# VatsalPandey0202/PointCloudRegistration

Hardware: AMD Instinct MI355X
Metric: TOF/PC pairs/sec (8192 pts) (higher is better)
Workload: dtype f32 xyz/features; f64 RANSAC/ICP; 1-term f16 MFMA screen (certified bound), f16x3-split MFMA screen for the rows it leaves, f64 exact re-rank; 1 GPU; C4: batch of augmented TOF/PC pairs (featNN+RANSAC+ICP+Chamfer); pairs_total=256, pairs_per_gpu=256, points=8192, feature_dim=32, streams_per_gpu=1, ransac=d=0.04 mutual n=3 edge0.9 dist0.04 (100000,0.999), icp=d=0.02 (1e-6,1e-6,30), parallelism=pair-sharded x1, inputs=resident in HBM (--full: host_resident is the PCIe-inclusive rate)

## Files before the change

### pointcloudregistration_amd/csrc/featnn_thresh.h

```cpp
#pragma once
#include <stdint.h>
#include <string.h>

#if defined(__HIPCC__)
#define PCR_THRESH_HD __host__ __device__
#else
#define PCR_THRESH_HD
#endif

namespace pcr {

PCR_THRESH_HD inline uint32_t thresh_bits_up(double t) {
    if (!(t == t)) return 0x7f800000u;
    if (!(t > 0.0)) return 0u;
    const float f = (float)t;
    uint32_t b;
    memcpy(&b, &f, sizeof(b));
    return (double)f < t ? b + 1u : b;
}

}
```

### pointcloudregistration_amd/csrc/featnn_thresh.hip

```cpp
#include "featnn_v5.h"
#include "featnn_thresh.h"
#include <stdlib.h>
#include <algorithm>
#include <cstdio>

namespace pcr {
namespace {

__device__ unsigned g_thresh_stat[2][3];

template <int S, bool kIdx>
__global__ __launch_bounds__(512) void featnn_thresh9(RowArgs5 a) {
    constexpr int NM = 2 * S + 1, NB = S, W = 8, RT = 2;
    const int nbp = gridDim.x / (8 * ((a.P + 7) >> 3));
    const int bid = blockIdx.x, xcd = bid & 7, slot = bid >> 3;
    const int p = (slot / nbp) * 8 + xcd, sl = slot % nbp;
    if (p >= a.P) return;
    const int nr = min(a.rcount[p], a.Rmax);
    const int m = count_of(a.n_cols, p, a.Cmax);
    const int nst = (((m + 31) >> 5) + 1) >> 1;
    const int nsl = min(nbp, nst);
    if (nr <= 0 || sl >= nsl) return;
    const int s0 = (int)((long long)nst * sl / nsl), s1 = (int)((long long)nst * (sl + 1) / nsl);
    const int wid = threadIdx.x >> 6, l = threadIdx.x & 63, h = l >> 5;
    const int ntl = (nr + 31) >> 5;
    const int *rl = a.rlist + (size_t)p * a.Rmax;
    const f16x8 *bimg = a.Bp + (size_t)p * a.ntc * NM * 64 + l;
    const float *ctp = a.cct + (size_t)p * a.ntc * 32;
    auto load = [&](int st, f16x8 (&Bf)[2][NB], f32x16 (&Cf)[2]) {
#pragma unroll
        for (int u = 0; u < 2; ++u) {
#pragma unroll
            for (int c = 0; c < NB; ++c) Bf[u][c] = bimg[((size_t)(2 * st + u) * NM + c) * 64];
            Cf[u] = colterms(ctp + (size_t)(2 * st + u) * 32, h);
        }
    };
    for (int t0 = wid * RT; t0 < ntl; t0 += W * RT) {
        size_t o[RT];
        unsigned B1[RT], thr[RT], am[RT];
        bool live[RT];
        int nh[RT];
        f16x8 A[RT][NB];
#pragma unroll
        for (int t = 0; t < RT; ++t) {
            const int k = (t0 + t) * 32 + (l & 31);
            const bool valid = k < nr;
            const int row = valid ? rl[k] : 0;
            o[t] = (size_t)p * a.Rmax + row;
            B1[t] = valid ? a.rec[o[t]].y : 0x7f800000u;
            thr[t] = 0u;
            live[t] = false;
            if (valid && B1[t] < 0x7f800000u) {
                const double bnd = row_bound_ct(a, p, row, a.rre[(size_t)p * a.ntr * 32 + row], 16 * S);
                thr[t] = thresh_bits_up((double)__uint_as_float(B1[t]) + bnd * (1.0 + 0x1p-20));
                live[t] = thr[t] < 0x7f800000u;
            }
            row_operand1<S>(a, p, row, valid, h, A[t]);
            am[t] = 0xffffffffu;
            nh[t] = 0;
        }
        f16x8 Bf[2][NB];
        f32x16 Cf[2];
        load(s0, Bf, Cf);
        for (int st = s0; st < s1; ++st) {
            f16x8 Bn[2][NB];
            f32x16 Cn[2];
            load(st + 1 < s1 ? st + 1 : st, Bn, Cn);
            f32x16 acc[RT][2];
#pragma unroll
            for (int c = 0; c < NB; ++c)
#pragma unroll
                for (int u = 0; u < 2; ++u)
#pragma unroll
                    for (int t = 0; t < RT; ++t)
                        acc[t][u] = __builtin_amdgcn_mfma_f32_32x32x16_f16(Bf[u][c], A[t][c],
                                                                           c == 0 ? Cf[u] : acc[t][u], 0, 0, 0);
#pragma unroll
            for (int t = 0; t < RT; ++t)
#pragma unroll
                for (int u = 0; u < 2; ++u) {
                    unsigned long long any = 0ull;
#pragma unroll
                    for (int r = 0; r < 16; ++r) any |= __ballot(fbits(acc[t][u][r]) <= thr[t]);
                    if (any == 0ull) continue;
#pragma unroll
                    for (int r = 0; r < 16; ++r) {
                        const unsigned v = fbits(acc[t][u][r]);
                        const int col = 32 * (2 * st + u) + 8 * (r >> 2) + 4 * h + (r & 3);
                        if (v <= thr[t] && live[t] && col < m) {
                            if (kIdx && v == B1[t]) am[t] = umin2(am[t], (unsigned)col);
                            if (nh[t] <= kThreshK) {
                                const unsigned pos = atomicAdd(reinterpret_cast<unsigned *>(a.rec + o[t]), 1u);
                                if (pos < (unsigned)kThreshK) a.cand[o[t] * kThreshK + pos] = col;
                            }
                            ++nh[t];
                        }
                    }
                }
#pragma unroll
            for (int u = 0; u < 2; ++u) {
#pragma unroll
                for (int c = 0; c < NB; ++c) Bf[u][c] = Bn[u][c];
                Cf[u] = Cn[u];
            }
        }
#pragma unroll
        for (int t = 0; t < RT; ++t)
            if (kIdx && am[t] != 0xffffffffu) atomicMin(reinterpret_cast<unsigned *>(a.rec + o[t]) + 2, am[t]);
    }
}

template <int DV, bool kIdx>
__global__ __launch_bounds__(256) void featnn_exact_cand(RowArgs5 a) {
    const int p = blockIdx.y;
    const int nr = min(a.rcount[p], a.Rmax);
    if (nr <= 0) return;
    if (blockIdx.x == 0 && threadIdx.x == 0) atomicAdd(a.fbctr + (kIdx ? 0 : 1), (unsigned long long)nr);
    const int m = count_of(a.n_cols, p, a.Cmax);
    const int *rl = a.rlist + (size_t)p * a.Rmax;
    const int c = threadIdx.x & 7, rr = threadIdx.x >> 3, D = a.D;
    const float4 open = make_float4(__builtin_inff(), __builtin_inff(), __builtin_inff(), 0.0f);
    for (int k0 = blockIdx.x * 32; k0 < nr; k0 += gridDim.x * 32) {
        const bool act = k0 + rr < nr;
        const int row = act ? rl[k0 + rr] : 0;
        const size_t o = (size_t)p * a.Rmax + row;
        const uint4 rc = act ? a.rec[o] : make_uint4(0u, 0x7f800000u, 0u, 1u);
        const int cnt = (int)min(rc.x, (unsigned)kThreshK + 1u);
        double best = __builtin_inf();
        int bj = 0x7fffffff;
        if (act && m > 0 && c < cnt && cnt <= kThreshK && rc.y < 0x7f800000u) {
            const int j = a.cand[o * kThreshK + c];
            const float *q = a.Xr + o * D, *y = a.Xc + ((size_t)p * a.Cmax + j) * D;
            float qf[DV], yf[DV];
            if (D == DV && (((uintptr_t)q | (uintptr_t)y) & 15) == 0) {
#pragma unroll
                for (int k = 0; k < DV; k += 4) {
                    const float4 u = *reinterpret_cast<const float4 *>(q + k), w = *reinterpret_cast<const float4 *>(y + k);
                    qf[k] = u.x; qf[k + 1] = u.y; qf[k + 2] = u.z; qf[k + 3] = u.w;
                    yf[k] = w.x; yf[k + 1] = w.y; yf[k + 2] = w.z; yf[k + 3] = w.w;
                }
            } else {
#pragma unroll
                for (int k = 0; k < DV; ++k) {
                    qf[k] = k < D ? q[k] : 0.0f;
                    yf[k] = k < D ? y[k] : 0.0f;
                }
            }
            double acc = 0.0;
#pragma unroll
            for (int k = 0; k < DV; ++k) {
                const double df = (double)qf[k] - (double)yf[k];
                acc = acc + df * df;
            }
            if (acc < best) { best = acc; bj = j; }
        }
#pragma unroll
        for (int x = 1; x < 8; x <<= 1) {
            const double ob = __shfl_xor(best, x, 64);
            const int oj = __shfl_xor(bj, x, 64);
            if (ob < best || (ob == best && oj < bj)) { best = ob; bj = oj; }
        }
        if (c != 0 || !act) continue;
        if (m == 0) {
            if constexpr (kIdx) {
                a.nn[o] = 0;
                a.nns[o] = 0;
                a.v[o] = __builtin_inf();
                a.e[o] = 0.0f;
            } else {
                a.wq[o] = open;
            }
            continue;
        }
        if constexpr (kIdx) a.nns[o] = rc.z < (unsigned)m ? (int)rc.z : 0;
        const bool over = bj == 0x7fffffff;
        if (a.dbg) {
            atomicAdd(&g_thresh_stat[kIdx ? 0 : 1][0], 1u);
            atomicMax(&g_thresh_stat[kIdx ? 0 : 1][1], rc.x);
            if (over) atomicAdd(&g_thresh_stat[kIdx ? 0 : 1][2], 1u);
        }
        if constexpr (kIdx) {
            if (over) {
                a.llist[(size_t)p * a.Rmax + atomicAdd(a.lcount + p, 1)] = row;
            } else {
                const double sc = (double)__uint_as_float(a.sc[p]);
                a.nn[o] = bj;
                a.v[o] = best * sc * sc;
                a.e[o] = 0.0f;
            }
        } else {
            a.wq[o] = open;
            if (!over) {
                a.nn[o] = bj;
                a.used[(size_t)p * (a.Rmax + 1) + row] = 2;
            }
        }
    }
}

}

static int thresh_blocks_per_pair(int P) {
    static const int forced = [] {
        const char *e = getenv("PCR_THRESH_SLICES");
        return e ? atoi(e) : 0;
    }();
    if (forced >= 1 && forced <= 128) return forced;
    return std::max(4, std::min(32, 1024 / std::max(P, 1)));
}

template <bool kIdx>
int launch_thresh9(const RowArgs5 &r0, int S, hipStream_t s) {
    RowArgs5 r = r0;
    static const bool dbg = getenv("PCR_THRESH_DEBUG") != nullptr;
    r.dbg = dbg ? 1 : 0;
    int rc = fallback_counter(&r.fbctr);
    if (rc != PCR_OK) return rc;
    const int nbp = thresh_blocks_per_pair(r.P);
    const dim3 grid((unsigned)(8LL * nbp * cdiv(r.P, 8)));
    if (S == 1) hipLaunchKernelGGL((featnn_thresh9<1, kIdx>), grid, dim3(512), 0, s, r);
    else hipLaunchKernelGGL((featnn_thresh9<2, kIdx>), grid, dim3(512), 0, s, r);
    PCR_LAUNCH_CHECK();
    const dim3 eg(std::min(8, cdiv(r.Rmax, 32)), r.P);
    if (S == 1) hipLaunchKernelGGL((featnn_exact_cand<16, kIdx>), eg, dim3(256), 0, s, r);
    else hipLaunchKernelGGL((featnn_exact_cand<32, kIdx>), eg, dim3(256), 0, s, r);
    PCR_LAUNCH_CHECK();
    if (dbg) {
        unsigned st[2][3];
        PCR_HIP_CHECK(hipStreamSynchronize(s));
        PCR_HIP_CHECK(hipMemcpyFromSymbol(st, HIP_SYMBOL(g_thresh_stat), sizeof(st)));
        const int d = kIdx ? 0 : 1;
        fprintf(stderr, "thresh pass %d: listed %u, max candidates %u, to the exact rescan %u\n", d + 1, st[d][0],
                st[d][1], st[d][2]);
        const unsigned z[3] = {0, 0, 0};
        PCR_HIP_CHECK(hipMemcpyToSymbol(HIP_SYMBOL(g_thresh_stat), z, sizeof(z), sizeof(z) * d));
    }
    return PCR_OK;
}

template int launch_thresh9<true>(const RowArgs5 &, int, hipStream_t);
template int launch_thresh9<false>(const RowArgs5 &, int, hipStream_t);

}
```

Measured before the change: 48730 pairs/s.

## Stage column tiles in LDS via async global_load_lds and batch candidate hits locally

The threshold-screen kernel now stages groups of column B-fragments and column terms into double-buffered shared memory with async global-to-LDS loads, so the eight waves of a block share one copy instead of each loading from global memory. Candidate hits are counted and stored in per-row LDS slots and flushed to global memory with one atomic per row per row-block, replacing a global atomic per hit. The hit scan first reduces each half of the accumulator to a minimum before balloting. The default number of blocks per pair also drops (256/P instead of 1024/P, minimum 1). This adds large LDS use and block-wide barriers, which may reduce occupancy.

```diff
diff --git a/pointcloudregistration_amd/csrc/featnn_thresh.h b/pointcloudregistration_amd/csrc/featnn_thresh.h
--- a/pointcloudregistration_amd/csrc/featnn_thresh.h
+++ b/pointcloudregistration_amd/csrc/featnn_thresh.h
@@ -19,4 +19,10 @@
     return (double)f < t ? b + 1u : b;
 }
 
+PCR_THRESH_HD inline int thresh_flush_count(uint32_t base, uint32_t local, int K) {
+    if (base >= (uint32_t)K) return 0;
+    const uint32_t room = (uint32_t)K - base;
+    return (int)(local < room ? local : room);
 }
+
+}
diff --git a/pointcloudregistration_amd/csrc/featnn_thresh.hip b/pointcloudregistration_amd/csrc/featnn_thresh.hip
--- a/pointcloudregistration_amd/csrc/featnn_thresh.hip
+++ b/pointcloudregistration_amd/csrc/featnn_thresh.hip
@@ -3,15 +3,42 @@
 #include <stdlib.h>
 #include <algorithm>
 #include <cstdio>
+#include <type_traits>
 
 namespace pcr {
 namespace {
 
 __device__ unsigned g_thresh_stat[2][3];
 
+#ifndef PCR_THRESH_G
+#define PCR_THRESH_G 16
+#endif
+#ifndef PCR_THRESH_PF
+#define PCR_THRESH_PF 1
+#endif
+constexpr int kThreshG = PCR_THRESH_G;
+
+__device__ __forceinline__ unsigned lds_add_rtn(unsigned addr, unsigned v) {
+    unsigned r;
+    asm volatile("ds_add_rtn_u32 %0, %1, %2\n\ts_waitcnt lgkmcnt(0)" : "=v"(r) : "v"(addr), "v"(v) : "memory");
+    return r;
+}
+__device__ __forceinline__ void lds_store(unsigned addr, int v) {
+    asm volatile("ds_write_b32 %0, %1\n\ts_waitcnt lgkmcnt(0)" : : "v"(addr), "v"(v) : "memory");
+}
+
 template <int S, bool kIdx>
 __global__ __launch_bounds__(512) void featnn_thresh9(RowArgs5 a) {
-    constexpr int NM = 2 * S + 1, NB = S, W = 8, RT = 2;
+    constexpr int NM = 2 * S + 1, NB = S, W = 8, RT = 2, G = kThreshG, GS = G / 2;
+    constexpr int kT = G * NB * 64;
+    constexpr int kRows = W * RT * 32;
+    static_assert(G % 2 == 0 && kRows == 512, "whole steps; the flush is one row per thread");
+    __shared__ __attribute__((aligned(16))) f16x8 Bs0[kT];
+    __shared__ __attribute__((aligned(16))) f16x8 Bs1[kT];
+    __shared__ __attribute__((aligned(16))) float Cs0[G * 32];
+    __shared__ __attribute__((aligned(16))) float Cs1[G * 32];
+    __shared__ unsigned hcnt[kRows];
+    __shared__ int hslot[kRows * kThreshK];
     const int nbp = gridDim.x / (8 * ((a.P + 7) >> 3));
     const int bid = blockIdx.x, xcd = bid & 7, slot = bid >> 3;
     const int p = (slot / nbp) * 8 + xcd, sl = slot % nbp;
@@ -22,28 +49,55 @@
     const int nsl = min(nbp, nst);
     if (nr <= 0 || sl >= nsl) return;
     const int s0 = (int)((long long)nst * sl / nsl), s1 = (int)((long long)nst * (sl + 1) / nsl);
+    const int ngr = (s1 - s0 + GS - 1) / GS;
     const int wid = threadIdx.x >> 6, l = threadIdx.x & 63, h = l >> 5;
     const int ntl = (nr + 31) >> 5;
     const int *rl = a.rlist + (size_t)p * a.Rmax;
     const f16x8 *bimg = a.Bp + (size_t)p * a.ntc * NM * 64 + l;
-    const float *ctp = a.cct + (size_t)p * a.ntc * 32;
-    auto load = [&](int st, f16x8 (&Bf)[2][NB], f32x16 (&Cf)[2]) {
-#pragma unroll
-        for (int u = 0; u < 2; ++u) {
-#pragma unroll
-            for (int c = 0; c < NB; ++c) Bf[u][c] = bimg[((size_t)(2 * st + u) * NM + c) * 64];
-            Cf[u] = colterms(ctp + (size_t)(2 * st + u) * 32, h);
+    const float *ctp = a.cct + (size_t)p * a.ntc * 32 + l;
+    auto issue = [&](auto bufc_, int grp) {
+        f16x8 *Bs = decltype(bufc_)::value ? Bs1 : Bs0;
+        float *Cs = decltype(bufc_)::value ? Cs1 : Cs0;
+        const int sg = s0 + grp * GS;
+        for (int c = wid; c < G * NB + GS; c += W) {
+            if (c >= G * NB) {
+                const int j = c - G * NB;
+                if (sg + j < s1)
+                    __builtin_amdgcn_global_load_lds(
+                        (const __attribute__((address_space(1))) void *)(ctp + (size_t)(sg + j) * 64),
+                        (__attribute__((address_space(3))) void *)(Cs + j * 64),
+                        4, 0, 0);
+                continue;
+            }
+            const int g = c / NB, cc = c - g * NB;
+            if (sg + (g >> 1) < s1)
+                __builtin_amdgcn_global_load_lds(
+                    (const __attribute__((address_space(1))) void *)(bimg + ((size_t)(2 * sg + g) * NM + cc) * 64),
+                    (__attribute__((address_space(3))) void *)(Bs + c * 64), 16, 0, 0);
         }
     };
-    for (int t0 = wid * RT; t0 < ntl; t0 += W * RT) {
+    auto min8 = [](const f32x16 &x, int q) {
+        unsigned c = umin2(umin2(fbits(x[8 * q]), fbits(x[8 * q + 1])), fbits(x[8 * q + 2]));
+        c = umin2(umin2(c, fbits(x[8 * q + 3])), fbits(x[8 * q + 4]));
+        c = umin2(umin2(c, fbits(x[8 * q + 5])), fbits(x[8 * q + 6]));
+        return umin2(c, fbits(x[8 * q + 7]));
+    };
+    for (int tb = 0; tb < ntl; tb += W * RT) {
+        hcnt[threadIdx.x] = 0u;
+        issue(std::integral_constant<int, 0>{}, 0);
+        const int nt = tb + wid + W < ntl ? 2 : (tb + wid < ntl ? 1 : 0);
         size_t o[RT];
         unsigned B1[RT], thr[RT], am[RT];
         bool live[RT];
-        int nh[RT];
+        int nh[RT], lr[RT];
+        unsigned ca[RT], sa[RT];
         f16x8 A[RT][NB];
 #pragma unroll
         for (int t = 0; t < RT; ++t) {
-            const int k = (t0 + t) * 32 + (l & 31);
+            lr[t] = (t * W + wid) * 32 + (l & 31);
+            ca[t] = (unsigned)(uintptr_t)(hcnt + lr[t]);
+            sa[t] = (unsigned)(uintptr_t)(hslot + lr[t] * kThreshK);
+            const int k = tb * 32 + lr[t];
             const bool valid = k < nr;
             const int row = valid ? rl[k] : 0;
             o[t] = (size_t)p * a.Rmax + row;
@@ -59,54 +113,98 @@
             am[t] = 0xffffffffu;
             nh[t] = 0;
         }
-        f16x8 Bf[2][NB];
-        f32x16 Cf[2];
-        load(s0, Bf, Cf);
-        for (int st = s0; st < s1; ++st) {
-            f16x8 Bn[2][NB];
-            f32x16 Cn[2];
-            load(st + 1 < s1 ? st + 1 : st, Bn, Cn);
-            f32x16 acc[RT][2];
-#pragma unroll
-            for (int c = 0; c < NB; ++c)
-#pragma unroll
-                for (int u = 0; u < 2; ++u)
-#pragma unroll
-                    for (int t = 0; t < RT; ++t)
-                        acc[t][u] = __builtin_amdgcn_mfma_f32_32x32x16_f16(Bf[u][c], A[t][c],
-                                                                           c == 0 ? Cf[u] : acc[t][u], 0, 0, 0);
-#pragma unroll
-            for (int t = 0; t < RT; ++t)
+        auto sweep = [&](auto ntc_, auto bufc_, int grp) {
+            constexpr int NT = decltype(ntc_)::value;
+            const f16x8 *Bs = decltype(bufc_)::value ? Bs1 : Bs0;
+            const float *Cb = decltype(bufc_)::value ? Cs1 : Cs0;
+            const int sg = s0 + grp * GS, ns = min(GS, s1 - sg);
+            const f16x8 *Bb = Bs + l;
+            auto load = [&](int j, f16x8 (&Bf)[2][NB], f32x16 (&Cf)[2]) {
 #pragma unroll
                 for (int u = 0; u < 2; ++u) {
-                    unsigned long long any = 0ull;
-#pragma unroll
-                    for (int r = 0; r < 16; ++r) any |= __ballot(fbits(acc[t][u][r]) <= thr[t]);
-                    if (any == 0ull) continue;
-#pragma unroll
-                    for (int r = 0; r < 16; ++r) {
-                        const unsigned v = fbits(acc[t][u][r]);
-                        const int col = 32 * (2 * st + u) + 8 * (r >> 2) + 4 * h + (r & 3);
-                        if (v <= thr[t] && live[t] && col < m) {
-                            if (kIdx && v == B1[t]) am[t] = umin2(am[t], (unsigned)col);
-                            if (nh[t] <= kThreshK) {
-                                const unsigned pos = atomicAdd(reinterpret_cast<unsigned *>(a.rec + o[t]), 1u);
-                                if (pos < (unsigned)kThreshK) a.cand[o[t] * kThreshK + pos] = col;
+#pragma unroll
+                    for (int c = 0; c < NB; ++c) Bf[u][c] = Bb[((2 * j + u) * NB + c) * 64];
+                    Cf[u] = colterms(Cb + (2 * j + u) * 32, h);
+                }
+            };
+            f16x8 Bf[2][NB];
+            f32x16 Cf[2];
+            if (PCR_THRESH_PF) load(0, Bf, Cf);
+            for (int j = 0; j < ns; ++j) {
+                const int st = sg + j;
+                f16x8 Bn[2][NB];
+                f32x16 Cn[2];
+                if (PCR_THRESH_PF) load(j + 1 < ns ? j + 1 : j, Bn, Cn);
+                else load(j, Bf, Cf);
+                f32x16 acc[NT][2];
+#pragma unroll
+                for (int c = 0; c < NB; ++c)
+#pragma unroll
+                    for (int u = 0; u < 2; ++u)
+#pragma unroll
+                        for (int t = 0; t < NT; ++t)
+                            acc[t][u] = __builtin_amdgcn_mfma_f32_32x32x16_f16(Bf[u][c], A[t][c],
+                                                                               c == 0 ? Cf[u] : acc[t][u], 0, 0, 0);
+#pragma unroll
+                for (int t = 0; t < NT; ++t)
+#pragma unroll
+                    for (int u = 0; u < 2; ++u) {
+                        const unsigned m0 = min8(acc[t][u], 0), m1 = min8(acc[t][u], 1);
+                        if (__ballot(umin2(m0, m1) <= thr[t]) == 0ull) continue;
+                        const bool half[2] = {__ballot(m0 <= thr[t]) != 0ull, __ballot(m1 <= thr[t]) != 0ull};
+#pragma unroll
+                        for (int r = 0; r < 16; ++r) {
+                            if (!half[r >> 3]) continue;
+                            const unsigned v = fbits(acc[t][u][r]);
+                            const int col = 32 * (2 * st + u) + 8 * (r >> 2) + 4 * h + (r & 3);
+                            if (v <= thr[t] && live[t] && col < m) {
+                                if (kIdx && v == B1[t]) am[t] = umin2(am[t], (unsigned)col);
+                                if (nh[t] <= kThreshK) {
+                                    const unsigned pos = lds_add_rtn(ca[t], 1u);
+                                    if (pos < (unsigned)kThreshK) lds_store(sa[t] + 4u * pos, col);
+                                }
+                                ++nh[t];
                             }
-                            ++nh[t];
                         }
                     }
+                if (PCR_THRESH_PF) {
+#pragma unroll
+                    for (int u = 0; u < 2; ++u) {
+#pragma unroll
+                        for (int c = 0; c < NB; ++c) Bf[u][c] = Bn[u][c];
+                        Cf[u] = Cn[u];
+                    }
                 }
-#pragma unroll
-            for (int u = 0; u < 2; ++u) {
-#pragma unroll
-                for (int c = 0; c < NB; ++c) Bf[u][c] = Bn[u][c];
-                Cf[u] = Cn[u];
-            }
+            }
+        };
+        asm volatile("s_waitcnt vmcnt(0)" ::: "memory");
+        __syncthreads();
+        auto group = [&](auto bufc_, int grp) {
+            constexpr int buf = decltype(bufc_)::value;
+            if (grp + 1 < ngr) issue(std::integral_constant<int, buf ^ 1>{}, grp + 1);
+            if (nt == 2) sweep(std::integral_constant<int, 2>{}, bufc_, grp);
+            else if (nt == 1) sweep(std::integral_constant<int, 1>{}, bufc_, grp);
+            asm volatile("s_waitcnt vmcnt(0)" ::: "memory");
+            __syncthreads();
+        };
+        for (int grp = 0; grp < ngr; grp += 2) {
+            group(std::integral_constant<int, 0>{}, grp);
+            if (grp + 1 < ngr) group(std::integral_constant<int, 1>{}, grp + 1);
         }
 #pragma unroll
         for (int t = 0; t < RT; ++t)
             if (kIdx && am[t] != 0xffffffffu) atomicMin(reinterpret_cast<unsigned *>(a.rec + o[t]) + 2, am[t]);
+        {
+            const int r = threadIdx.x, k = tb * 32 + r;
+            const unsigned lc = hcnt[r];
+            if (k < nr && lc != 0u) {
+                const size_t oo = (size_t)p * a.Rmax + rl[k];
+                const unsigned base = atomicAdd(reinterpret_cast<unsigned *>(a.rec + oo), lc);
+                const int n = thresh_flush_count(base, lc, kThreshK);
+                for (int i = 0; i < n; ++i) a.cand[oo * kThreshK + base + i] = hslot[r * kThreshK + i];
+            }
+        }
+        __syncthreads();
     }
 }
 
@@ -206,7 +304,7 @@
         return e ? atoi(e) : 0;
     }();
     if (forced >= 1 && forced <= 128) return forced;
-    return std::max(4, std::min(32, 1024 / std::max(P, 1)));
+    return std::max(1, std::min(32, 256 / std::max(P, 1)));
 }
 
 template <bool kIdx>
```

Result: faster. 50300 pairs/s (median of 6 runs) (+3.2%).
